# openai/Video-Pre-Training

Measured on NVIDIA H100. Metric: frames/sec MinecraftPolicy fwd, 128x128x3 BxT=128x128, higher is better.
Workload: dtype bf16

## Files before the change

video-pre-training_b200/csrc/conv_zp.cuh:

```cuda
#pragma once
#include "common.cuh"
#include "gemm_tc.cuh"

namespace vpt {

static int g_cz_dbg = 0;

constexpr int kCzThreads = 384;
constexpr int kCzMaxBStages = 8;
constexpr int kCzProducerRegs = 24, kCzMmaRegs = 240;

constexpr int kCzBarOrder = 1, kCzBarStg = 3, kCzBarWg = 5;

struct ConvZpParams {
    long long Q;
    int H, W, Wp, FS;
    int N, block_n, num_n_tiles, cin, cin_blocks;
    int a_box_rows, a_boxes, a_stage_bytes, b_stages;
    int dbg;
    int bo;
    long long num_m_tiles;
    const float* mr;
    const float* S1;
    const float* S2;
    int relu;
    const __nv_bfloat16* residual;
    __nv_bfloat16* out;
    float* stat_part;
    const float* Ef;
    const float* res_scale;
    const float* res_shift;
};

template <int BN>
__device__ __forceinline__ void cz_mma_k16(float (&acc)[BN / 2], uint64_t a_desc, uint64_t b_desc, uint32_t accumulate) {
    if constexpr (BN == 128)
        wgmma_n128<0, 0>(acc, a_desc, b_desc, accumulate);
    else
        wgmma_n64<0, 0>(acc, a_desc, b_desc, accumulate);
}

template <int BN>
__global__ void __launch_bounds__(kCzThreads, 1)
conv3x3_zp_kernel(const __grid_constant__ CUtensorMap tmA, const __grid_constant__ CUtensorMap tmB, const ConvZpParams p) {
    static_assert(BN == 64 || BN == 128, "BN is 64 or 128");
    pdl_sync();
    extern __shared__ uint8_t smem_raw[];
    const uint32_t raw = smem_u32(smem_raw);
    uint8_t* smem = smem_raw + (((raw + 1023u) & ~1023u) - raw);
    constexpr uint32_t b_stage_bytes = (uint32_t)BN * kBlockK * 2;
    uint8_t* smem_a = smem;
    uint8_t* smem_b = smem + 2 * (size_t)p.a_stage_bytes;
    float* stg = reinterpret_cast<float*>(smem_b + (size_t)p.b_stages * b_stage_bytes);
    uint64_t* bars = reinterpret_cast<uint64_t*>(reinterpret_cast<uint8_t*>(stg) + kStgBytes);
    uint64_t* a_full = bars;
    uint64_t* a_empty = bars + 2;
    uint64_t* b_full = bars + 4;
    uint64_t* b_empty = bars + 4 + kCzMaxBStages;

    const int warp = threadIdx.x >> 5;
    const int lane = threadIdx.x & 31;

    if (warp == 8 && lane == 0) {
        tma_prefetch_desc(&tmA);
        tma_prefetch_desc(&tmB);
        for (int i = 0; i < 2; ++i) {
            mbar_init(&a_full[i], 1);
            mbar_init(&a_empty[i], 1);
        }
        for (int i = 0; i < p.b_stages; ++i) {
            mbar_init(&b_full[i], 1);
            mbar_init(&b_empty[i], 1);
        }
        fence_barrier_init();
    }
    __syncthreads();

    const int num_tiles = (int)(p.num_m_tiles * p.num_n_tiles);
    const int tile_begin = (int)blockIdx.x;
    const int tile_step = (int)gridDim.x;
    const int halo = p.Wp + 1;

    if (warp >= 8) {
        setmaxnreg_dec<kCzProducerRegs>();
        if (warp == 8 && lane == 0) {
            int stage = 0;
            uint32_t phase = 0;
            bool ok = true;
            for (int tile = tile_begin; tile < num_tiles && ok; tile += tile_step) {
                const int m_tile = tile / p.num_n_tiles;
                const int span0 = m_tile * kBlockM - halo;
                for (int cb = 0; cb < p.cin_blocks; ++cb) {
                    if (!(ok = mbar_wait(&a_empty[stage], phase ^ 1u, 0x110u))) break;
                    mbar_expect_tx(&a_full[stage], (uint32_t)p.a_stage_bytes);
                    uint8_t* sa = smem_a + (size_t)stage * p.a_stage_bytes;
                    for (int b = 0; b < p.a_boxes; ++b)
                        tma_load_2d(sa + (size_t)b * p.a_box_rows * 128, &tmA, &a_full[stage], cb * kBlockK, span0 + b * p.a_box_rows);
                    advance(stage, phase, 2);
                }
            }
        } else if (warp == 9 && lane == 0) {
            int stage = 0;
            uint32_t phase = 0;
            bool ok = true;
            for (int tile = tile_begin; tile < num_tiles && ok; tile += tile_step) {
                const int n0 = (tile % p.num_n_tiles) * BN;
                for (int cb = 0; cb < p.cin_blocks && ok; ++cb) {
                    for (int tap = 0; tap < 9; ++tap) {
                        if (!(ok = mbar_wait(&b_empty[stage], phase ^ 1u, 0x120u))) break;
                        mbar_expect_tx(&b_full[stage], b_stage_bytes);
                        tma_load_2d(smem_b + (size_t)stage * b_stage_bytes, &tmB, &b_full[stage], tap * p.cin + cb * kBlockK, n0);
                        advance(stage, phase, p.b_stages);
                    }
                }
            }
        }
        return;
    }

    setmaxnreg_inc<kCzMmaRegs>();
    const int wg = warp >> 2;
    const int wwarp = warp & 3;
    float* my_row = stg + (size_t)(wwarp * 32 + lane) * kStgPitch;
    const int nchunks = BN >> 5;
    const int c_half = (nchunks + 1) >> 1;
    const int P = p.num_n_tiles * 2;
    const bool res_vec = (((uintptr_t)p.residual | (uintptr_t)p.res_scale | (uintptr_t)p.res_shift) & 15) == 0;
    const int b_per_tile = 9 * p.cin_blocks;
    for (int s = wg; tile_begin + s * tile_step < num_tiles; s += 2) {
        const int tile = tile_begin + s * tile_step;
        const bool has_next = tile + tile_step < num_tiles;
        const int m_tile = tile / p.num_n_tiles;
        const int n_tile = tile % p.num_n_tiles;
        const int n0 = n_tile * BN;
        const long long a_it = (long long)s * p.cin_blocks, b_it = (long long)s * b_per_tile;
        int astage = (int)(a_it & 1), bstage = (int)(b_it % p.b_stages);
        uint32_t aphase = (uint32_t)((a_it >> 1) & 1), bphase = (uint32_t)((b_it / p.b_stages) & 1);

        if (s > 0) named_bar_sync(kCzBarOrder + wg, 256);
        float frag[2][BN / 2];
        bool ok = true;
        int prev_b = -1, prev_a = -1;
        for (int cb = 0; cb < p.cin_blocks && ok; ++cb) {
            if (!(ok = mbar_wait(&a_full[astage], aphase, 0x310u))) break;
            const uint32_t a_base = smem_u32(smem_a + (size_t)astage * p.a_stage_bytes);
#pragma unroll 1
            for (int tap = 0; tap < 9; ++tap) {
                if (!(ok = mbar_wait(&b_full[bstage], bphase, 0x320u))) break;
                const uint32_t b_addr = smem_u32(smem_b + (size_t)bstage * b_stage_bytes);
                const int row_off = (tap / 3) * p.Wp + (tap % 3);
                const uint32_t a_addr = a_base + (uint32_t)row_off * 128u;
                const uint64_t a_bo = p.bo ? ((uint64_t)((a_addr >> 7) & 7u) << 49) : 0ull;
                wgmma_fence();
#pragma unroll
                for (int k = 0; k < kBlockK / 16; ++k) {
                    const uint32_t acc = (uint32_t)((cb | tap | k) != 0);
                    const uint64_t bd = gmma_desc_sw128(b_addr + k * 32);
                    cz_mma_k16<BN>(frag[0], gmma_desc_sw128(a_addr + k * 32) | a_bo, bd, acc);
                    cz_mma_k16<BN>(frag[1], gmma_desc_sw128(a_addr + 64u * 128u + k * 32) | a_bo, bd, acc);
                }
                wgmma_commit();
                wgmma_wait<1>();
                if ((threadIdx.x & 127) == 0) {
                    if (prev_b >= 0) mbar_arrive(&b_empty[prev_b]);
                    if (prev_a >= 0) mbar_arrive(&a_empty[prev_a]);
                }
                prev_a = -1;
                prev_b = bstage;
                advance(bstage, bphase, p.b_stages);
            }
            prev_a = astage;
            advance(astage, aphase, 2);
        }
        if (has_next) named_bar_arrive(kCzBarOrder + (wg ^ 1), 256);
        wgmma_wait<0>();
#pragma unroll
        for (int h = 0; h < 2; ++h) wgmma_reg_fence(frag[h]);
        if ((threadIdx.x & 127) == 0) {
            if (prev_b >= 0) mbar_arrive(&b_empty[prev_b]);
            if (prev_a >= 0) mbar_arrive(&a_empty[prev_a]);
        }
        if (!ok) {
            if (has_next) named_bar_arrive(kCzBarStg + (wg ^ 1), 256);
            break;
        }

        if (s > 0) named_bar_sync(kCzBarStg + wg, 256);
#pragma unroll
        for (int h = 0; h < 2; ++h) wgmma_frag_store(frag[h], stg + (size_t)h * 64 * kStgPitch, kStgPitch, 0);
        named_bar_sync(kCzBarWg + wg, 128);

        const int q = m_tile * kBlockM + wwarp * 32 + lane;
        const bool row_ok = q < p.Q;
        const int f = q / p.FS;
        const int r = q - f * p.FS;
        const int y = r / p.Wp, x = r - y * p.Wp;
        const bool interior = row_ok && (y < p.H) && (x < p.W);
        float ga = 1.f, gb = 0.f;
        if (p.mr != nullptr && interior) {
            const float mean = __ldg(p.mr + 2 * f), rstd = __ldg(p.mr + 2 * f + 1);
            ga = rstd;
            gb = rstd * mean;
        }
        const int cy = (y == 0) ? 0 : ((y == p.H - 1) ? 2 : 1);
        const int cx = (x == 0) ? 0 : ((x == p.W - 1) ? 2 : 1);
        const int cls = interior ? cy * 3 + cx : 0;
        const float* s1row = p.S1 ? p.S1 + (size_t)cls * p.N : nullptr;
        const float* s2row = p.S2 ? p.S2 + (size_t)cls * p.N : nullptr;
        if (p.Ef) {
            s1row = nullptr;
            s2row = p.Ef + ((size_t)(interior ? f : 0) * 9 + cls) * p.N;
        }
        const float* rarow = (p.res_scale && interior) ? p.res_scale + (size_t)f * p.N : nullptr;
        const float* rbrow = (p.res_scale && interior) ? p.res_shift + (size_t)f * p.N : nullptr;
        float st_s0 = 0.f, st_ss0 = 0.f, st_s1 = 0.f, st_ss1 = 0.f;

        const int qw = m_tile * kBlockM + wwarp * 32;
        float* wrows = stg + (size_t)(wwarp * 32) * kStgPitch;
        const int seg = lane & 3;
#pragma unroll 1
        for (int c = 0; c < (p.dbg == 2 ? 0 : nchunks); ++c) {
            const int g = c < c_half ? 0 : 1;
            const int nb = n0 + c * 32;
            const int lim = min(32, min(BN - c * 32, p.N - nb));
            if (lim <= 0) break;
            const bool full = (lim == 32) && ((p.N & 7) == 0) && res_vec;
            uint32_t acc[32];
            float v[32];
            uint32_t pk[16];
            if (full) {
                stg_ld_32(my_row + c * 32, acc);
                __syncwarp();
                if (p.residual != nullptr) {
#pragma unroll
                    for (int k = 0; k < 4; ++k) {
                        const int rr = 8 * k + (lane >> 2);
                        if (qw + rr < p.Q)
                            reinterpret_cast<uint4*>(wrows + (size_t)rr * kStgPitch + c * 32)[seg] =
                                __ldg(reinterpret_cast<const uint4*>(p.residual + (size_t)(qw + rr) * p.N + nb) + seg);
                    }
                    __syncwarp();
                }
                if (row_ok) {
                    if (!interior) {
#pragma unroll
                        for (int j = 0; j < 16; ++j) pk[j] = 0u;
                    } else {
#pragma unroll
                        for (int qq = 0; qq < 8; ++qq) {
                            float4 a1 = s1row ? __ldg(reinterpret_cast<const float4*>(s1row + nb) + qq) : make_float4(0, 0, 0, 0);
                            float4 a2 = s2row ? __ldg(reinterpret_cast<const float4*>(s2row + nb) + qq) : make_float4(0, 0, 0, 0);
                            v[4 * qq + 0] = fmaf(ga, __uint_as_float(acc[4 * qq + 0]), fmaf(-gb, a1.x, a2.x));
                            v[4 * qq + 1] = fmaf(ga, __uint_as_float(acc[4 * qq + 1]), fmaf(-gb, a1.y, a2.y));
                            v[4 * qq + 2] = fmaf(ga, __uint_as_float(acc[4 * qq + 2]), fmaf(-gb, a1.z, a2.z));
                            v[4 * qq + 3] = fmaf(ga, __uint_as_float(acc[4 * qq + 3]), fmaf(-gb, a1.w, a2.w));
                        }
                        if (p.relu == 1) {
#pragma unroll
                            for (int j = 0; j < 32; ++j) v[j] = fmaxf(v[j], 0.f);
                        }
                        if (p.residual != nullptr) {
                            const uint4* rp = reinterpret_cast<const uint4*>(my_row + c * 32);
#pragma unroll
                            for (int qq = 0; qq < 4; ++qq) {
                                const uint4 rr = rp[qq];
                                const float r8[8] = {bf16_lo(rr.x), bf16_hi(rr.x), bf16_lo(rr.y), bf16_hi(rr.y),
                                                     bf16_lo(rr.z), bf16_hi(rr.z), bf16_lo(rr.w), bf16_hi(rr.w)};
                                if (rarow) {
                                    const float4* ra4 = reinterpret_cast<const float4*>(rarow + nb) + 2 * qq;
                                    const float4* rb4 = reinterpret_cast<const float4*>(rbrow + nb) + 2 * qq;
                                    const float4 a0 = __ldg(ra4), a1 = __ldg(ra4 + 1), b0 = __ldg(rb4), b1 = __ldg(rb4 + 1);
                                    const float ra[8] = {a0.x, a0.y, a0.z, a0.w, a1.x, a1.y, a1.z, a1.w};
                                    const float rb[8] = {b0.x, b0.y, b0.z, b0.w, b1.x, b1.y, b1.z, b1.w};
#pragma unroll
                                    for (int j = 0; j < 8; ++j) v[8 * qq + j] += fmaf(ra[j], r8[j], rb[j]);
                                } else {
#pragma unroll
                                    for (int j = 0; j < 8; ++j) v[8 * qq + j] += r8[j];
                                }
                            }
                        }
                        if (p.relu == 2) {
#pragma unroll
                            for (int j = 0; j < 32; ++j) v[j] = fmaxf(v[j], 0.f);
                        }
#pragma unroll
                        for (int j = 0; j < 16; ++j) pk[j] = pack_bf16(v[2 * j], v[2 * j + 1]);
                        if (p.stat_part) {
                            float s_ = g ? st_s1 : st_s0, ss_ = g ? st_ss1 : st_ss0;
#pragma unroll
                            for (int j = 0; j < 16; ++j) {
                                const float lo = bf16_lo(pk[j]), hi = bf16_hi(pk[j]);
                                s_ += lo; ss_ = fmaf(lo, lo, ss_);
                                s_ += hi; ss_ = fmaf(hi, hi, ss_);
                            }
                            if (g) { st_s1 = s_; st_ss1 = ss_; } else { st_s0 = s_; st_ss0 = ss_; }
                        }
                    }
#pragma unroll
                    for (int qq = 0; qq < 4; ++qq)
                        reinterpret_cast<uint4*>(my_row + c * 32 + 16)[qq] = make_uint4(pk[4 * qq], pk[4 * qq + 1], pk[4 * qq + 2], pk[4 * qq + 3]);
                }
                __syncwarp();
                if (p.dbg != 1) {
#pragma unroll
                    for (int k = 0; k < 4; ++k) {
                        const int rr = 8 * k + (lane >> 2);
                        if (qw + rr < p.Q)
                            reinterpret_cast<uint4*>(p.out + (size_t)(qw + rr) * p.N + nb)[seg] =
                                reinterpret_cast<const uint4*>(wrows + (size_t)rr * kStgPitch + c * 32 + 16)[seg];
                    }
                }
                continue;
            }
            if (!row_ok) continue;
            stg_ld_32(my_row + c * 32, acc);
            __nv_bfloat16* op = p.out + (size_t)q * p.N + nb;
            if (!interior) {
                for (int j = 0; j < lim; ++j) op[j] = __float2bfloat16_rn(0.f);
                continue;
            }
#pragma unroll
            for (int j = 0; j < 32; ++j) {
                float a1 = 0.f, a2 = 0.f;
                if (j < lim) {
                    if (s1row) a1 = __ldg(s1row + nb + j);
                    if (s2row) a2 = __ldg(s2row + nb + j);
                }
                v[j] = fmaf(ga, __uint_as_float(acc[j]), fmaf(-gb, a1, a2));
            }
            if (p.relu == 1) {
#pragma unroll
                for (int j = 0; j < 32; ++j) v[j] = fmaxf(v[j], 0.f);
            }
            if (p.residual != nullptr) {
                const __nv_bfloat16* rp = p.residual + (size_t)q * p.N + nb;
#pragma unroll
                for (int j = 0; j < 32; ++j)
                    if (j < lim) v[j] += rarow ? fmaf(__ldg(rarow + nb + j), __bfloat162float(rp[j]), __ldg(rbrow + nb + j)) : __bfloat162float(rp[j]);
            }
            if (p.relu == 2) {
#pragma unroll
                for (int j = 0; j < 32; ++j) v[j] = fmaxf(v[j], 0.f);
            }
#pragma unroll
            for (int j = 0; j < 16; ++j) pk[j] = pack_bf16(v[2 * j], v[2 * j + 1]);
            if (p.stat_part) {
                float s_ = g ? st_s1 : st_s0, ss_ = g ? st_ss1 : st_ss0;
#pragma unroll
                for (int j = 0; j < 16; ++j) {
                    const float lo = bf16_lo(pk[j]), hi = bf16_hi(pk[j]);
                    if (2 * j < lim) { s_ += lo; ss_ = fmaf(lo, lo, ss_); }
                    if (2 * j + 1 < lim) { s_ += hi; ss_ = fmaf(hi, hi, ss_); }
                }
                if (g) { st_s1 = s_; st_ss1 = ss_; } else { st_s0 = s_; st_ss0 = ss_; }
            }
            if (p.dbg != 1) {
#pragma unroll
                for (int j = 0; j < 32; ++j)
                    if (j < lim) op[j] = __float2bfloat16_rn(v[j]);
            }
        }
        if (has_next) named_bar_arrive(kCzBarStg + (wg ^ 1), 256);
        if (p.stat_part && row_ok)
            reinterpret_cast<float4*>(p.stat_part)[((size_t)q * P + n_tile * 2) >> 1] = make_float4(st_s0, st_ss0, st_s1, st_ss1);
    }
}

}

namespace vpt {
static inline void conv_zp_block_n(long long Q, int N, int* bn, int* nt) {
    choose_block_n(N, bn, nt);
    const long long tiles = (Q + kBlockM - 1) / kBlockM;
    if (tiles * *nt >= 64 || *bn == 64) return;
    *bn = 64;
    *nt = (N + 63) / 64;
}
}

extern "C" int vpt_conv3x3_zp(const vpt_conv_zp_args* a, void* stream) {
    using namespace vpt;
    VPT_CHECK(a && a->x && a->w && a->out, "vpt_conv3x3_zp: null operand");
    const int H = a->H, W = a->W, C = a->Cin, N = a->Cout;
    VPT_CHECK(a->F > 0 && H >= 2 && W >= 2 && C > 0 && C % 64 == 0 && N > 0 && N % 16 == 0,
              "vpt_conv3x3_zp: need F>0, H,W>=2, Cin %% 64 == 0, Cout %% 16 == 0 (F=%d H=%d W=%d Cin=%d Cout=%d)", a->F, H, W, C, N);
    VPT_CHECK(W <= 182, "vpt_conv3x3_zp: W=%d too wide (at most 182: two input spans of 128 + 2*(W+2) rows must fit in shared memory)", W);
    VPT_CHECK(((uintptr_t)a->x & 15) == 0 && ((uintptr_t)a->w & 15) == 0 && ((uintptr_t)a->out & 15) == 0, "vpt_conv3x3_zp: pointers must be 16-byte aligned");
    ConvZpParams p;
    memset(&p, 0, sizeof(p));
    p.H = H; p.W = W; p.Wp = W + 1; p.FS = (H + 1) * (W + 1);
    p.Q = (long long)a->F * p.FS;
    VPT_CHECK(p.Q <= 2147483647LL - kBlockM, "vpt_conv3x3_zp: too many rows for 32-bit row indices and TMA coordinates");
    p.N = N; p.cin = C; p.cin_blocks = C / 64;
    conv_zp_block_n(p.Q, N, &p.block_n, &p.num_n_tiles);
    p.num_m_tiles = (p.Q + kBlockM - 1) / kBlockM;
    const int span = kBlockM + 2 * (p.Wp + 1);
    p.a_boxes = (span + 255) / 256;
    p.a_box_rows = ((span + p.a_boxes - 1) / p.a_boxes + 7) / 8 * 8;
    VPT_CHECK(p.a_box_rows <= 256, "vpt_conv3x3_zp: span does not fit the TMA box limit");
    p.a_stage_bytes = p.a_boxes * p.a_box_rows * 128;
    const uint32_t b_stage_bytes = (uint32_t)p.block_n * kBlockK * 2;
    const size_t fixed_bytes = 1024 + 2 * (size_t)p.a_stage_bytes + kStgBytes + (4 + 2 * kCzMaxBStages) * 8;
    int bst = (int)((227 * 1024 - (long long)fixed_bytes) / b_stage_bytes);
    if (bst > kCzMaxBStages) bst = kCzMaxBStages;
    VPT_CHECK(bst >= 2, "vpt_conv3x3_zp: not enough shared memory for the weight pipeline (W=%d Cout=%d)", W, N);
    p.b_stages = bst;
    const size_t smem_bytes = fixed_bytes + (size_t)bst * b_stage_bytes;

    CUtensorMap tmA, tmB;
    {
        cuuint64_t dims[2] = {(cuuint64_t)C, (cuuint64_t)p.Q};
        cuuint64_t strides[1] = {(cuuint64_t)C * 2};
        cuuint32_t box[2] = {64, (cuuint32_t)p.a_box_rows};
        int r = make_tmap_bf16(&tmA, a->x, 2, dims, strides, box);
        if (r) return r;
    }
    {
        cuuint64_t dims[2] = {(cuuint64_t)9 * C, (cuuint64_t)N};
        cuuint64_t strides[1] = {(cuuint64_t)9 * C * 2};
        cuuint32_t box[2] = {64, (cuuint32_t)p.block_n};
        int r = make_tmap_bf16(&tmB, a->w, 2, dims, strides, box);
        if (r) return r;
    }
    VPT_CHECK(!(a->mr && !a->S1 && !a->Ef), "vpt_conv3x3_zp: mr given without S1 (or Ef)");
    VPT_CHECK(!a->Ef || a->mr, "vpt_conv3x3_zp: Ef needs mr = (0, rstd) per frame");
    VPT_CHECK(!a->res_scale == !a->res_shift && (!a->res_scale || a->residual) && (!a->res_scale || N % 8 == 0),
              "vpt_conv3x3_zp: res_scale / res_shift come as a pair, with a residual, Cout %% 8 == 0");
    p.mr = a->mr; p.S1 = a->mr ? a->S1 : nullptr; p.S2 = a->S2; p.relu = a->relu;
    p.residual = reinterpret_cast<const __nv_bfloat16*>(a->residual);
    p.out = reinterpret_cast<__nv_bfloat16*>(a->out);
    p.stat_part = a->stat_part;
    p.Ef = a->Ef; p.res_scale = a->res_scale; p.res_shift = a->res_shift;
    p.dbg = g_cz_dbg;
    p.bo = g_dbg_bo > 0 ? 1 : 0;

    static bool attr_set = false;
    if (!attr_set) {
        VPT_CUDA(cudaFuncSetAttribute(conv3x3_zp_kernel<64>, cudaFuncAttributeMaxDynamicSharedMemorySize, 227 * 1024));
        VPT_CUDA(cudaFuncSetAttribute(conv3x3_zp_kernel<128>, cudaFuncAttributeMaxDynamicSharedMemorySize, 227 * 1024));
        attr_set = true;
    }
    const long long tiles = p.num_m_tiles * p.num_n_tiles;
    long long grid = num_sms();
    if (grid <= 0) grid = 132;
    if (grid > tiles) grid = tiles;
    if (p.block_n == 64)
        launch_k(conv3x3_zp_kernel<64>, dim3((unsigned)grid), dim3(kCzThreads), smem_bytes, (cudaStream_t)stream, tmA, tmB, p);
    else
        launch_k(conv3x3_zp_kernel<128>, dim3((unsigned)grid), dim3(kCzThreads), smem_bytes, (cudaStream_t)stream, tmA, tmB, p);
    VPT_LAUNCH_CHECK();
    return VPT_OK;
}

extern "C" int vpt_set_conv_pair_mode(int32_t on) {
    vpt::g_cz_dbg = (on & 0xff) >> 4;
    return VPT_OK;
}

extern "C" int vpt_set_conv_swap_mode(int32_t on) {
    (void)on;
    return VPT_OK;
}

extern "C" int64_t vpt_conv_zp_t_stat_floats(int32_t F, int32_t H, int32_t W, int32_t Cout) {
    (void)F; (void)H; (void)W; (void)Cout;
    return 0;
}

extern "C" int vpt_conv_zp_t_stats_finalize(const float* part, float* mr, int32_t F, int32_t H, int32_t W, float eps, void* stream) {
    (void)part; (void)mr; (void)F; (void)H; (void)W; (void)eps; (void)stream;
    vpt::set_error("vpt_conv_zp_t_stats_finalize: no convolution kernel of this build emits per-tile partials (vpt_conv_zp_t_stat_floats is 0)");
    return VPT_ERR_ARG;
}

extern "C" int vpt_conv_zp_stat_parts(int32_t F, int32_t H, int32_t W, int32_t Cout) {
    const long long Q = (long long)F * (H + 1) * (W + 1);
    int bn, nt;
    vpt::conv_zp_block_n(Q, Cout, &bn, &nt);
    return nt * 2;
}
```

Baseline: 26400.

## Release staging buffer early via register copy and per-warp swizzled bounce buffer

```diff
diff --git a/video-pre-training_b200/csrc/conv_zp.cuh b/video-pre-training_b200/csrc/conv_zp.cuh
--- a/video-pre-training_b200/csrc/conv_zp.cuh
+++ b/video-pre-training_b200/csrc/conv_zp.cuh
@@ -9,6 +9,7 @@
 constexpr int kCzThreads = 384;
 constexpr int kCzMaxBStages = 8;
 constexpr int kCzProducerRegs = 24, kCzMmaRegs = 240;
+constexpr uint32_t kCzBounceBytes = 8u * 32u * 64u;
 
 constexpr int kCzBarOrder = 1, kCzBarStg = 3, kCzBarWg = 5;
 
@@ -50,7 +51,8 @@
     uint8_t* smem = smem_raw + (((raw + 1023u) & ~1023u) - raw);
     constexpr uint32_t b_stage_bytes = (uint32_t)BN * kBlockK * 2;
     uint8_t* smem_a = smem;
-    uint8_t* smem_b = smem + 2 * (size_t)p.a_stage_bytes;
+    uint8_t* bounce = smem + 2 * (size_t)p.a_stage_bytes;
+    uint8_t* smem_b = bounce + kCzBounceBytes;
     float* stg = reinterpret_cast<float*>(smem_b + (size_t)p.b_stages * b_stage_bytes);
     uint64_t* bars = reinterpret_cast<uint64_t*>(reinterpret_cast<uint8_t*>(stg) + kStgBytes);
     uint64_t* a_full = bars;
@@ -121,9 +123,11 @@
     setmaxnreg_inc<kCzMmaRegs>();
     const int wg = warp >> 2;
     const int wwarp = warp & 3;
-    float* my_row = stg + (size_t)(wwarp * 32 + lane) * kStgPitch;
-    const int nchunks = BN >> 5;
-    const int c_half = (nchunks + 1) >> 1;
+    const float* my_row = stg + (size_t)(wwarp * 32 + lane) * kStgPitch;
+    uint8_t* wbounce = bounce + (size_t)warp * 32 * 64;
+    auto bpiece = [wbounce](int r, int piece) { return reinterpret_cast<uint4*>(wbounce + r * 64) + (piece ^ ((r >> 1) & 3)); };
+    constexpr int nchunks = BN / 32;
+    constexpr int c_half = (nchunks + 1) / 2;
     const int P = p.num_n_tiles * 2;
     const bool res_vec = (((uintptr_t)p.residual | (uintptr_t)p.res_scale | (uintptr_t)p.res_shift) & 15) == 0;
     const int b_per_tile = 9 * p.cin_blocks;
@@ -138,7 +142,7 @@
         uint32_t aphase = (uint32_t)((a_it >> 1) & 1), bphase = (uint32_t)((b_it / p.b_stages) & 1);
 
         if (s > 0) named_bar_sync(kCzBarOrder + wg, 256);
-        float frag[2][BN / 2];
+        float frag[2][BN / 2] = {};
         bool ok = true;
         int prev_b = -1, prev_a = -1;
         for (int cb = 0; cb < p.cin_blocks && ok; ++cb) {
@@ -189,6 +193,10 @@
 #pragma unroll
         for (int h = 0; h < 2; ++h) wgmma_frag_store(frag[h], stg + (size_t)h * 64 * kStgPitch, kStgPitch, 0);
         named_bar_sync(kCzBarWg + wg, 128);
+        uint32_t row[nchunks][32];
+#pragma unroll
+        for (int c = 0; c < nchunks; ++c) stg_ld_32(my_row + c * 32, row[c]);
+        if (has_next) named_bar_arrive(kCzBarStg + (wg ^ 1), 256);
 
         const int q = m_tile * kBlockM + wwarp * 32 + lane;
         const bool row_ok = q < p.Q;
@@ -216,28 +224,25 @@
         float st_s0 = 0.f, st_ss0 = 0.f, st_s1 = 0.f, st_ss1 = 0.f;
 
         const int qw = m_tile * kBlockM + wwarp * 32;
-        float* wrows = stg + (size_t)(wwarp * 32) * kStgPitch;
         const int seg = lane & 3;
-#pragma unroll 1
-        for (int c = 0; c < (p.dbg == 2 ? 0 : nchunks); ++c) {
+#pragma unroll
+        for (int c = 0; c < nchunks; ++c) {
             const int g = c < c_half ? 0 : 1;
             const int nb = n0 + c * 32;
             const int lim = min(32, min(BN - c * 32, p.N - nb));
-            if (lim <= 0) break;
+            if (p.dbg == 2 || lim <= 0) break;
             const bool full = (lim == 32) && ((p.N & 7) == 0) && res_vec;
-            uint32_t acc[32];
+            const uint32_t (&acc)[32] = row[c];
             float v[32];
             uint32_t pk[16];
             if (full) {
-                stg_ld_32(my_row + c * 32, acc);
                 __syncwarp();
                 if (p.residual != nullptr) {
 #pragma unroll
                     for (int k = 0; k < 4; ++k) {
                         const int rr = 8 * k + (lane >> 2);
                         if (qw + rr < p.Q)
-                            reinterpret_cast<uint4*>(wrows + (size_t)rr * kStgPitch + c * 32)[seg] =
-                                __ldg(reinterpret_cast<const uint4*>(p.residual + (size_t)(qw + rr) * p.N + nb) + seg);
+                            *bpiece(rr, seg) = __ldg(reinterpret_cast<const uint4*>(p.residual + (size_t)(qw + rr) * p.N + nb) + seg);
                     }
                     __syncwarp();
                 }
@@ -260,10 +265,9 @@
                             for (int j = 0; j < 32; ++j) v[j] = fmaxf(v[j], 0.f);
                         }
                         if (p.residual != nullptr) {
-                            const uint4* rp = reinterpret_cast<const uint4*>(my_row + c * 32);
 #pragma unroll
                             for (int qq = 0; qq < 4; ++qq) {
-                                const uint4 rr = rp[qq];
+                                const uint4 rr = *bpiece(lane, qq);
                                 const float r8[8] = {bf16_lo(rr.x), bf16_hi(rr.x), bf16_lo(rr.y), bf16_hi(rr.y),
                                                      bf16_lo(rr.z), bf16_hi(rr.z), bf16_lo(rr.w), bf16_hi(rr.w)};
                                 if (rarow) {
@@ -298,23 +302,19 @@
                         }
                     }
 #pragma unroll
-                    for (int qq = 0; qq < 4; ++qq)
-                        reinterpret_cast<uint4*>(my_row + c * 32 + 16)[qq] = make_uint4(pk[4 * qq], pk[4 * qq + 1], pk[4 * qq + 2], pk[4 * qq + 3]);
+                    for (int qq = 0; qq < 4; ++qq) *bpiece(lane, qq) = make_uint4(pk[4 * qq], pk[4 * qq + 1], pk[4 * qq + 2], pk[4 * qq + 3]);
                 }
                 __syncwarp();
                 if (p.dbg != 1) {
 #pragma unroll
                     for (int k = 0; k < 4; ++k) {
                         const int rr = 8 * k + (lane >> 2);
-                        if (qw + rr < p.Q)
-                            reinterpret_cast<uint4*>(p.out + (size_t)(qw + rr) * p.N + nb)[seg] =
-                                reinterpret_cast<const uint4*>(wrows + (size_t)rr * kStgPitch + c * 32 + 16)[seg];
+                        if (qw + rr < p.Q) reinterpret_cast<uint4*>(p.out + (size_t)(qw + rr) * p.N + nb)[seg] = *bpiece(rr, seg);
                     }
                 }
                 continue;
             }
             if (!row_ok) continue;
-            stg_ld_32(my_row + c * 32, acc);
             __nv_bfloat16* op = p.out + (size_t)q * p.N + nb;
             if (!interior) {
                 for (int j = 0; j < lim; ++j) op[j] = __float2bfloat16_rn(0.f);
@@ -361,7 +361,6 @@
                     if (j < lim) op[j] = __float2bfloat16_rn(v[j]);
             }
         }
-        if (has_next) named_bar_arrive(kCzBarStg + (wg ^ 1), 256);
         if (p.stat_part && row_ok)
             reinterpret_cast<float4*>(p.stat_part)[((size_t)q * P + n_tile * 2) >> 1] = make_float4(st_s0, st_ss0, st_s1, st_ss1);
     }
@@ -370,10 +369,28 @@
 }
 
 namespace vpt {
-static inline void conv_zp_block_n(long long Q, int N, int* bn, int* nt) {
+struct CzSmem {
+    int a_boxes, a_box_rows, a_stage_bytes;
+    size_t fixed_bytes;
+};
+static inline CzSmem conv_zp_smem(int W) {
+    CzSmem m;
+    const int span = kBlockM + 2 * (W + 2);
+    m.a_boxes = (span + 255) / 256;
+    m.a_box_rows = ((span + m.a_boxes - 1) / m.a_boxes + 7) / 8 * 8;
+    m.a_stage_bytes = m.a_boxes * m.a_box_rows * 128;
+    m.fixed_bytes = 1024 + 2 * (size_t)m.a_stage_bytes + kCzBounceBytes + kStgBytes + (4 + 2 * kCzMaxBStages) * 8;
+    return m;
+}
+static inline int conv_zp_b_stages(size_t fixed_bytes, int bn) {
+    const int bst = (int)((227 * 1024 - (long long)fixed_bytes) / ((long long)bn * kBlockK * 2));
+    return bst < kCzMaxBStages ? bst : kCzMaxBStages;
+}
+static inline void conv_zp_block_n(long long Q, int W, int N, int* bn, int* nt) {
     choose_block_n(N, bn, nt);
     const long long tiles = (Q + kBlockM - 1) / kBlockM;
-    if (tiles * *nt >= 64 || *bn == 64) return;
+    const bool wide = conv_zp_b_stages(conv_zp_smem(W).fixed_bytes, 128) < 2;
+    if (*bn == 64 || (tiles * *nt >= 64 && !wide)) return;
     *bn = 64;
     *nt = (N + 63) / 64;
 }
@@ -393,20 +410,17 @@
     p.Q = (long long)a->F * p.FS;
     VPT_CHECK(p.Q <= 2147483647LL - kBlockM, "vpt_conv3x3_zp: too many rows for 32-bit row indices and TMA coordinates");
     p.N = N; p.cin = C; p.cin_blocks = C / 64;
-    conv_zp_block_n(p.Q, N, &p.block_n, &p.num_n_tiles);
+    conv_zp_block_n(p.Q, W, N, &p.block_n, &p.num_n_tiles);
     p.num_m_tiles = (p.Q + kBlockM - 1) / kBlockM;
-    const int span = kBlockM + 2 * (p.Wp + 1);
-    p.a_boxes = (span + 255) / 256;
-    p.a_box_rows = ((span + p.a_boxes - 1) / p.a_boxes + 7) / 8 * 8;
+    const CzSmem sm = conv_zp_smem(W);
+    p.a_boxes = sm.a_boxes;
+    p.a_box_rows = sm.a_box_rows;
     VPT_CHECK(p.a_box_rows <= 256, "vpt_conv3x3_zp: span does not fit the TMA box limit");
-    p.a_stage_bytes = p.a_boxes * p.a_box_rows * 128;
-    const uint32_t b_stage_bytes = (uint32_t)p.block_n * kBlockK * 2;
-    const size_t fixed_bytes = 1024 + 2 * (size_t)p.a_stage_bytes + kStgBytes + (4 + 2 * kCzMaxBStages) * 8;
-    int bst = (int)((227 * 1024 - (long long)fixed_bytes) / b_stage_bytes);
-    if (bst > kCzMaxBStages) bst = kCzMaxBStages;
+    p.a_stage_bytes = sm.a_stage_bytes;
+    const int bst = conv_zp_b_stages(sm.fixed_bytes, p.block_n);
     VPT_CHECK(bst >= 2, "vpt_conv3x3_zp: not enough shared memory for the weight pipeline (W=%d Cout=%d)", W, N);
     p.b_stages = bst;
-    const size_t smem_bytes = fixed_bytes + (size_t)bst * b_stage_bytes;
+    const size_t smem_bytes = sm.fixed_bytes + (size_t)bst * p.block_n * kBlockK * 2;
 
     CUtensorMap tmA, tmB;
     {
@@ -477,6 +491,6 @@
 extern "C" int vpt_conv_zp_stat_parts(int32_t F, int32_t H, int32_t W, int32_t Cout) {
     const long long Q = (long long)F * (H + 1) * (W + 1);
     int bn, nt;
-    vpt::conv_zp_block_n(Q, Cout, &bn, &nt);
+    vpt::conv_zp_block_n(Q, W, Cout, &bn, &nt);
     return nt * 2;
 }
```

New measurement: 27070 (median of 6 runs). 1.03x the previous value.
